# openmm/NNPOps

Hardware: AMD Instinct MI355X
Metric: AEV+forces evaluations/sec (ANI-2x symmetry functions, energy+gradient), 10k-atom periodic box (higher is better)
Workload: dtype f32

## Files before the change

### include/nnpops_hip.h

```cpp
#ifndef NNPOPS_HIP_H
#define NNPOPS_HIP_H

#include <stdint.h>

#ifdef __cplusplus
extern "C" {
#endif

typedef enum {
    NNPOPS_OK = 0,
    NNPOPS_ERR_INVALID_ARGUMENT = -1,
    NNPOPS_ERR_HIP = -2,
    NNPOPS_ERR_UNSUPPORTED = -3,
    NNPOPS_ERR_CAPACITY = -4,
    NNPOPS_ERR_NO_DEVICE = -5
} nnpops_status;

const char* nnpops_last_error(void);
const char* nnpops_version(void);
int nnpops_device_count(void);

typedef struct nnpops_ani* nnpops_ani_t;

int nnpops_ani_create(nnpops_ani_t* out, int num_atoms, int num_species, float radial_cutoff, float angular_cutoff,
// ... 1 lines not shown
                      int num_angular, const float* angular_eta_rs_zeta_ths, int torchani, int device);
int nnpops_ani_destroy(nnpops_ani_t h);
int nnpops_ani_set_stream(nnpops_ani_t h, void* stream);

int nnpops_ani_compute(nnpops_ani_t h, const float* positions, const float* box, float* radial, float* angular);
int nnpops_ani_backprop(nnpops_ani_t h, const float* radial_deriv, const float* angular_deriv, float* position_deriv);
int nnpops_ani_compute_strided(nnpops_ani_t h, const float* positions, const float* box, float* radial, int radial_ld,
                               float* angular, int angular_ld);
int nnpops_ani_backprop_strided(nnpops_ani_t h, const float* radial_deriv, int radial_ld, const float* angular_deriv,
                                int angular_ld, float* position_deriv);
int nnpops_ani_backprop_box_strided(nnpops_ani_t h, const float* positions, const float* box, const float* radial_deriv, int radial_ld,
                                    const float* angular_deriv, int angular_ld, float* position_deriv, float* box_deriv);
int nnpops_ani_tangent_strided(nnpops_ani_t h, const float* position_tangent, float* radial_tangent, int radial_ld,
                               float* angular_tangent, int angular_ld);
int nnpops_ani_check(nnpops_ani_t h, int* max_radial_neighbors, int* max_angular_neighbors);
int nnpops_ani_overflow_word(nnpops_ani_t h, const int32_t** word);
int nnpops_ani_read_overflow(nnpops_ani_t h, int32_t* value);
int nnpops_ani_read_grid(nnpops_ani_t h, int32_t* out);
int nnpops_ani_describe(nnpops_ani_t h, char* text, int capacity);
int nnpops_ani_check_begin(nnpops_ani_t h);
int nnpops_ani_check_begin_with(nnpops_ani_t h, const int32_t** word, int32_t** publish_to, int32_t* stamp);
int nnpops_ani_check_end(nnpops_ani_t h);
int nnpops_ani_set_neighbor_algorithm(nnpops_ani_t h, int algorithm);

int nnpops_ani_set_molecules(nnpops_ani_t h, int num_molecules, const int32_t* molecule_offsets);

enum {
    NNPOPS_ANI_K_NEIGHBORS = 0,
    NNPOPS_ANI_K_RADIAL_FWD = 1,
    NNPOPS_ANI_K_ANGULAR_FWD = 2,
    NNPOPS_ANI_K_RADIAL_BWD = 3,
    NNPOPS_ANI_K_ANGULAR_BWD = 4,
    NNPOPS_ANI_K_CELL_GRID = 5,
    NNPOPS_ANI_NUM_KERNELS = 6
};
int nnpops_ani_enable_timing(nnpops_ani_t h, int enable);
int nnpops_ani_set_timing_stride(nnpops_ani_t h, int every);
int nnpops_ani_get_timing(nnpops_ani_t h, double* total_ms, int* launches);
int nnpops_ani_timing_overhead(nnpops_ani_t h, double* ms);
int nnpops_ani_set_timing_merge(nnpops_ani_t h, int merge);

typedef struct nnpops_cfconv_neighbors* nnpops_cfconv_neighbors_t;
typedef struct nnpops_cfconv* nnpops_cfconv_t;

int nnpops_cfconv_neighbors_create(nnpops_cfconv_neighbors_t* out, int num_atoms, float cutoff, int periodic, int device);
int nnpops_cfconv_neighbors_destroy(nnpops_cfconv_neighbors_t h);
// ... 202 lines not shown
```

### nnpops_amd/capi.py

```python
import ctypes as C
import os

import numpy as np
import torch

_HERE = os.path.dirname(os.path.abspath(__file__))
LIB_PATH = os.path.join(_HERE, "libnnpops_hip.so")

OK = 0
ERR_CAPACITY = -4

SIGNATURES = {
    "nnpops_last_error": (C.c_char_p, []),
    "nnpops_version": (C.c_char_p, []),
    "nnpops_device_count": (C.c_int, []),
    "nnpops_ani_create": (C.c_int, [C.POINTER(C.c_void_p), C.c_int, C.c_int, C.c_float, C.c_float, C.c_int, C.c_void_p,
                                    C.c_int, C.c_void_p, C.c_int, C.c_void_p, C.c_int, C.c_int]),
    "nnpops_ani_destroy": (C.c_int, [C.c_void_p]),
    "nnpops_ani_set_stream": (C.c_int, [C.c_void_p, C.c_void_p]),
    "nnpops_ani_compute": (C.c_int, [C.c_void_p, C.c_void_p, C.c_void_p, C.c_void_p, C.c_void_p]),
    "nnpops_ani_backprop": (C.c_int, [C.c_void_p, C.c_void_p, C.c_void_p, C.c_void_p]),
    "nnpops_ani_compute_strided": (C.c_int, [C.c_void_p, C.c_void_p, C.c_void_p, C.c_void_p, C.c_int, C.c_void_p, C.c_int]),
    "nnpops_ani_backprop_strided": (C.c_int, [C.c_void_p, C.c_void_p, C.c_int, C.c_void_p, C.c_int, C.c_void_p]),
    "nnpops_ani_backprop_box_strided": (C.c_int, [C.c_void_p, C.c_void_p, C.c_void_p, C.c_void_p, C.c_int, C.c_void_p, C.c_int, C.c_void_p,
                                                  C.c_void_p]),
    "nnpops_ani_tangent_strided": (C.c_int, [C.c_void_p, C.c_void_p, C.c_void_p, C.c_int, C.c_void_p, C.c_int]),
    "nnpops_ani_check": (C.c_int, [C.c_void_p, C.POINTER(C.c_int), C.POINTER(C.c_int)]),
    "nnpops_ani_check_begin": (C.c_int, [C.c_void_p]),
    "nnpops_ani_check_end": (C.c_int, [C.c_void_p]),
    "nnpops_ani_set_neighbor_algorithm": (C.c_int, [C.c_void_p, C.c_int]),
    "nnpops_ani_set_molecules": (C.c_int, [C.c_void_p, C.c_int, C.c_void_p]),
    "nnpops_ani_enable_timing": (C.c_int, [C.c_void_p, C.c_int]),
    "nnpops_ani_set_timing_stride": (C.c_int, [C.c_void_p, C.c_int]),
    "nnpops_ani_get_timing": (C.c_int, [C.c_void_p, C.POINTER(C.c_double), C.POINTER(C.c_int)]),
    "nnpops_ani_timing_overhead": (C.c_int, [C.c_void_p, C.POINTER(C.c_double)]),
    "nnpops_ani_overflow_word": (C.c_int, [C.c_void_p, C.POINTER(C.c_void_p)]),
    "nnpops_ani_read_overflow": (C.c_int, [C.c_void_p, C.POINTER(C.c_int32)]),
    "nnpops_ani_read_grid": (C.c_int, [C.c_void_p, C.POINTER(C.c_int32)]),
    "nnpops_ani_describe": (C.c_int, [C.c_void_p, C.c_char_p, C.c_int]),
    "nnpops_ani_check_begin_with": (C.c_int, [C.c_void_p, C.POINTER(C.c_void_p), C.POINTER(C.c_void_p), C.POINTER(C.c_int32)]),
    "nnpops_ani_set_timing_merge": (C.c_int, [C.c_void_p, C.c_int]),
    "nnpops_cfconv_neighbors_create": (C.c_int, [C.POINTER(C.c_void_p), C.c_int, C.c_float, C.c_int, C.c_int]),
    "nnpops_cfconv_neighbors_destroy": (C.c_int, [C.c_void_p]),
    "nnpops_cfconv_neighbors_set_stream": (C.c_int, [C.c_void_p, C.c_void_p]),
    "nnpops_cfconv_neighbors_build": (C.c_int, [C.c_void_p, C.c_void_p, C.c_void_p]),
    "nnpops_cfconv_neighbors_check": (C.c_int, [C.c_void_p, C.POINTER(C.c_int)]),
    "nnpops_cfconv_neighbors_export": (C.c_int, [C.c_void_p, C.c_int, C.c_void_p, C.c_void_p]),
    "nnpops_cfconv_neighbors_read_grid": (C.c_int, [C.c_void_p, C.POINTER(C.c_int32)]),
    "nnpops_cfconv_create": (C.c_int, [C.POINTER(C.c_void_p), C.c_int, C.c_int, C.c_int, C.c_float, C.c_int, C.c_float,
                                       C.c_int, C.c_void_p, C.c_void_p, C.c_void_p, C.c_void_p, C.c_int]),
    "nnpops_cfconv_destroy": (C.c_int, [C.c_void_p]),
    "nnpops_cfconv_set_stream": (C.c_int, [C.c_void_p, C.c_void_p]),
    "nnpops_cfconv_compute": (C.c_int, [C.c_void_p, C.c_void_p, C.c_void_p, C.c_void_p, C.c_void_p, C.c_void_p]),
# ... 183 lines not shown
        self.angular_width = self.num_species * (self.num_species + 1) // 2 * self.num_angular

    def __del__(self):
        h = getattr(self, "_h", None)
        if h:
            self._lib.nnpops_ani_destroy(h)
            self._h = None

    def set_molecules(self, molecule_offsets):
        if molecule_offsets is None:
            _check(self._lib.nnpops_ani_set_molecules(self._h, 0, None))
            self.num_molecules = 0
            return
        off = np.ascontiguousarray(molecule_offsets, dtype=np.int32)
        _check(self._lib.nnpops_ani_set_molecules(self._h, int(off.shape[0]) - 1, off.ctypes.data_as(C.c_void_p)))
        self.num_molecules = int(off.shape[0]) - 1

    def _box_shape(self):
        return (self.num_molecules, 3, 3) if self.num_molecules > 0 else (3, 3)

    def set_neighbor_algorithm(self, algorithm):
        _check(self._lib.nnpops_ani_set_neighbor_algorithm(self._h, int(algorithm)))

    def compute(self, positions, box=None, radial=None, angular=None, check=True):
        _dev_f32(positions, "positions", (self.num_atoms, 3))
        if self.periodic:
            if box is None:
                raise ValueError("periodic evaluator needs box vectors")
            _dev_f32(box, "box", self._box_shape())
        if radial is None:
            radial = torch.empty((self.num_atoms, self.radial_width), dtype=torch.float32, device=positions.device)
        if angular is None:
            angular = torch.empty((self.num_atoms, self.angular_width), dtype=torch.float32, device=positions.device)
        _check(self._lib.nnpops_ani_set_stream(self._h, _stream_ptr(positions.device)))
        for _ in range(8):
            _check(self._lib.nnpops_ani_compute(self._h, _ptr(positions), _ptr(box if self.periodic else None),
                                                _ptr(radial), _ptr(angular)))
            if not check:
                break
            code = self._lib.nnpops_ani_check(self._h, None, None)
            if code == OK:
                break
            if code != ERR_CAPACITY:
                _check(code)
        else:
            raise NNPOpsHipError(ERR_CAPACITY, "neighbour buffers kept overflowing")
# ... 1028 lines not shown
```

### nnpops_amd/csrc/ani.hip

```cpp
#include <algorithm>
#include <cmath>
#include <cstdlib>
#include <cstring>
#include <vector>

#include "ani_kernels.h"
#include "ani_fallback_kernels.h"
#include "ani_angular_mfma.h"
#include "ani_angular_bwd.h"
#include "ani_angular_generic.h"
#include "ani_radial_bwd.h"
#include "ani_build_forward.h"
#include "ani_box_grad.h"
#include "ani_tangent.h"
#include "celllist_host.h"

using namespace nnpops;

constexpr int kRbwdLatencyAtoms = 8192;
constexpr int kFuseAtoms = 4096;
struct nnpops_ani {
    AniParams hp{};
    AngularConsts ac{};
    AniParams* d_params = nullptr;
// ... 43 lines not shown
    int last_compact = -1;
    bool fwd_row_via_lds = true;
    int fwd_occ = 7;
    bool fwd_dynamic = false;
    int nstreams = 1;
    hipStream_t side[3] = {nullptr, nullptr, nullptr};
    hipEvent_t ev_fork = nullptr, ev_join[3] = {nullptr, nullptr, nullptr};
    bool can_split = false;
    int bwd_atoms_per_group = 1;
    int store_mode = 3;
    bool occ6 = false;
    int backward_kernel = 1;
    int fwd_atoms_per_group = 1;
    int* d_cnt_a = nullptr;
    int* d_cnt_ro = nullptr;
    double* d_box_partials = nullptr;
    int* d_status = nullptr;
    int* h_status = nullptr;
    int* h_status_dev = nullptr;
    int check_stamp = 0;
    bool check_pending = false;
    CellList cells;
    bool cells_disabled = false;
    int cap = 0;
    bool cap_fitted = false;
    int cap_angular = 0;
    int tile = 32;
    bool compact_bwd = false;
    bool computed = false;
    int ld_radial = 0, ld_angular = 0;
    bool last_used_cells = false;
    int* d_work_order = nullptr;
    bool work_order_valid = false;
    unsigned char* d_class_tile = nullptr;
    struct BwdClass { int tile, w0, nw; bool two_waves; };
    std::vector<BwdClass> bwd_classes;
    bool bwd_by_class = true;
    bool bwd_two_waves = false;
    double mean_triples = 0;
    int bwd_class_min = 512;
    int bwd_class_atoms = 16384;
    int cell_atoms = 1800;
    int lpt = 2;
    int backprop_stamp = 0;
    unsigned timing_mask = 0;
    int timing_every = 1;
// ... 474 lines not shown
        if (h->mfma_ok) {
            while (hp.fwd_split < 8 && (int)live.size() * hp.fwd_split * 2 <= kFwdSlots) hp.fwd_split *= 2;
            for (size_t b = 0; b < live.size(); b++)
                for (int p = 0; p < hp.fwd_split; p++) hp.fwd_slot_bucket[b * hp.fwd_split + p] = live[b];
        }
        for (int c = 0; c < kMaxAngularFns; c++) hp.m_of_c[c] = -1;
        h->fwd_identity = num_angular == h->nfrp * h->nfzp;
        for (int m = 0; m < num_angular; m++) {
            hp.m_of_c[hp.c_of_m[m]] = m;
            if (hp.c_of_m[m] != m) h->fwd_identity = false;
        }
        hp.fwd_zero_shift = 0;
        while ((4 << hp.fwd_zero_shift) < num_angular && hp.fwd_zero_shift < 6) hp.fwd_zero_shift++;
        h->fwd_identity = h->fwd_identity && num_angular <= 256;
        h->forward_kernel = h->mfma_ok ? 2 : -1;
        if (const char* e = std::getenv("NNPOPS_ANI_FWD_CHUNK")) { h->fwd_chunk = std::min(512, std::max(64, (std::atoi(e) + 15) / 16 * 16)); h->fwd_chunk_forced = true; }
        if (const char* e = std::getenv("NNPOPS_ANI_FUSE")) h->fuse_forward = std::atoi(e) != 0 ? 1 : 0;
        if (const char* e = std::getenv("NNPOPS_ANI_LPT")) h->lpt = std::atoi(e);
        if (const char* e = std::getenv("NNPOPS_ANI_CELL_ATOMS")) h->cell_atoms = std::max(1, std::atoi(e));
        if (const char* e = std::getenv("NNPOPS_ANI_RBWD")) h->rbwd_lanes = std::atoi(e) != 0;
        if (const char* e = std::getenv("NNPOPS_ANI_SCATTER")) h->scatter_mode = std::atoi(e) != 0 ? 1 : 0;
        h->cells.fine = 1;
        if (const char* e = std::getenv("NNPOPS_ANI_FINE_GRID")) h->cells.fine = std::atoi(e) != 0;
        if (const char* e = std::getenv("NNPOPS_ANI_FWD_ROWLDS")) h->fwd_row_via_lds = std::atoi(e) != 0;
        if (const char* e = std::getenv("NNPOPS_ANI_FWD_OCC")) h->fwd_occ = std::atoi(e);
        {
            std::vector<double> frac(num_species, 0.0);
            for (int i = 0; i < num_atoms; i++) frac[atom_species[i]] += 1.0 / num_atoms;
            double fmax = 0;
            for (int a = 0; a < num_species; a++)
                for (int b = a; b < num_species; b++) fmax = std::max(fmax, frac[a] * frac[b] * (a == b ? 1.0 : 2.0));
            h->fwd_dynamic = h->mfma_ok && 32.0 * fmax / hp.fwd_split > 3.0;
        }
        if (const char* e = std::getenv("NNPOPS_ANI_FWD_DYN")) h->fwd_dynamic = std::atoi(e) != 0;
        if (const char* e = std::getenv("NNPOPS_ANI_STREAMS")) h->nstreams = std::max(1, std::min(4, std::atoi(e)));
        if (const char* e = std::getenv("NNPOPS_ANI_BWD_APG")) h->bwd_atoms_per_group = std::atoi(e);
        if (const char* e = std::getenv("NNPOPS_ANI_STORE")) h->store_mode = std::atoi(e) & 3;
        if (const char* e = std::getenv("NNPOPS_ANI_OCC")) h->occ6 = std::atoi(e) >= 6;
        if (const char* e = std::getenv("NNPOPS_ANI_BACKWARD")) { h->backward_kernel = std::min(4, std::max(0, std::atoi(e))); h->backward_forced = true; }
        if (const char* e = std::getenv("NNPOPS_ANI_FWD_WPA")) h->fwd_waves_per_atom = std::atoi(e) == 1 ? 1 : 2;
        if (const char* e = std::getenv("NNPOPS_ANI_FWD_APG")) h->fwd_atoms_per_group = std::max(1, std::atoi(e));
    }
    h->device = device;
    h->cap = 128;
    h->cap_angular = 32;
    if (const char* e = std::getenv("NNPOPS_ANI_CAP")) h->cap = std::max(16, std::atoi(e) & ~15);
// ... 130 lines not shown
            first[m + 1] = (int)blocks.size();
        }
        dev_free(h->d_mol_blocks); dev_free(h->d_mol_first_block); dev_free(h->d_mol_partials);
        h->num_mol_blocks = 0;
        if ((rc = dev_alloc(&h->d_mol_blocks, blocks.size()))) return rc;
        if ((rc = dev_alloc(&h->d_mol_first_block, first.size()))) return rc;
        if ((rc = dev_alloc(&h->d_mol_partials, 9 * blocks.size()))) return rc;
        NNPOPS_HIP_TRY(hipMemcpy(h->d_mol_blocks, blocks.data(), sizeof(int2) * blocks.size(), hipMemcpyHostToDevice));
        NNPOPS_HIP_TRY(hipMemcpy(h->d_mol_first_block, first.data(), sizeof(int) * first.size(), hipMemcpyHostToDevice));
        h->num_mol_blocks = (int)blocks.size();
    }
    h->num_molecules = num_molecules;
    h->computed = false;
    return NNPOPS_OK;
}

int nnpops_ani_set_neighbor_algorithm(nnpops_ani_t h, int algorithm) {
    NNPOPS_REQUIRE(h != nullptr, "NULL handle");
    NNPOPS_REQUIRE(algorithm >= 0 && algorithm <= 2, "algorithm must be 0 (auto), 1 (all pairs) or 2 (cell list)");
    h->algorithm = algorithm;
    return NNPOPS_OK;
}

int nnpops_ani_compute(nnpops_ani_t h, const float* positions, const float* box, float* radial, float* angular) {
    return nnpops_ani_compute_strided(h, positions, box, radial, 0, angular, 0);
}

int nnpops_ani_compute_strided(nnpops_ani_t h, const float* positions, const float* box, float* radial, int radial_ld,
                               float* angular, int angular_ld) {
    NNPOPS_REQUIRE(h != nullptr, "NULL handle");
    {
        const int wr = h->hp.S * h->hp.nR, wa = h->hp.NB * h->hp.nA;
        NNPOPS_REQUIRE((radial_ld == 0 || radial_ld >= wr) && (angular_ld == 0 || angular_ld >= wa),
                       "row strides must be 0 (dense) or at least the row widths (%d, %d)", wr, wa);
        h->ld_radial = radial_ld ? radial_ld : wr;
        h->ld_angular = angular_ld ? angular_ld : wa;
    }
    NNPOPS_REQUIRE(positions && radial && angular, "NULL device pointer");
    NNPOPS_REQUIRE(!h->hp.periodic || box, "periodic handle needs box vectors");
    DeviceGuard guard(h->device);
    if (!guard.ok) return fail(NNPOPS_ERR_HIP, "cannot select device %d", h->device);
    const int N = h->hp.N;
    const bool per = h->hp.periodic;

    const int lds_bw = (int)((builder_lds_bytes(h->cap, h->hp.S, h->hp.NB) + 15) & ~(size_t)15);
    const int wpg_b = waves_per_group(lds_bw);
    const size_t lds_b = (size_t)lds_bw * wpg_b;
    const dim3 ablock(64 * wpg_b);
    const bool use_cells = !h->d_segment && (h->algorithm == 2 || (h->algorithm == 0 && N >= h->cell_atoms && !h->cells_disabled));
    h->last_used_cells = use_cells;
    if (use_cells) {
        KernelTimer timer(h, NNPOPS_ANI_K_CELL_GRID);
        launch_cell_build(h->stream, N, positions, box, per, h->hp.rcr, h->d_species, h->cells);
    }
    h->can_split = !h->generic && h->forward_kernel == 2 && h->backward_kernel >= 1 &&
                   pair_backward_fits(h);
    Span spans[4];
    const int nspans = make_spans(h, spans);
    int rc = fork_streams(h, spans, nspans);
    if (rc != NNPOPS_OK) return rc;
    for (int q = 0; q < nspans; q++) {
        const Span& sp = spans[q];
        const dim3 sgrid(div_up(sp.nw, wpg_b));
        h->last_fused_build = build_forward_fused(h, angular);
        if (h->last_fused_build) {
            KernelTimer timer(h, NNPOPS_ANI_K_NEIGHBORS, sp.stream);
            KernelTimer merged_timer(h, NNPOPS_ANI_K_NEIGHBORS, sp.stream, true);
            const BuildInputs in{box, h->cells.grid, h->cells.cell_start, h->cells.sorted_cell, h->cells.sorted_pos, h->cells.hist, positions, h->d_species,
                                 h->d_segment, use_cells ? 1 : 0, per ? 1 : 0};
            const BuildOutputs out{h->d_nbr, h->d_recA, h->d_recB, h->d_ids, h->d_tri, h->d_cnt_a, h->d_cnt_ro, h->d_cnt_pos, h->d_status, radial, h->ld_radial};
            rc = h->hp.torchani ? launch_build_forward<true>(h, in, out, angular, sp) : launch_build_forward<false>(h, in, out, angular, sp);
            if (rc != NNPOPS_OK) return rc;
            continue;
        }
        KernelTimer merged_timer(h, NNPOPS_ANI_K_NEIGHBORS, sp.stream, true);
// ... 290 lines not shown
                const int tile = tiles[pending];
                h->bwd_classes.push_back({tile, start, end - start, end > start && triples / (end - start) >= 200.0});
                for (int q = start; q < end; q++) tile_of[perm[q]] = (unsigned char)std::min(255, tile);
                start = end;
                pending = c + 1;
            }
        }
        NNPOPS_HIP_TRY(hipMemcpyAsync(h->d_class_tile, tile_of.data(), tile_of.size(), hipMemcpyHostToDevice, h->stream));
        NNPOPS_HIP_TRY(hipStreamSynchronize(h->stream));
        h->work_order_valid = true;
    }
    h->tile = std::min(32, std::max(8, st[kStatMaxAngular]));
    h->compact_bwd = st[kStatMaxAngular] <= h->tile && h->tile >= 16 &&
                     h->tile * (h->tile + 1) + h->tile * (h->tile - 1) / 2 >= h->cap_angular * 4 + 12;
    if (max_radial_neighbors) *max_radial_neighbors = st[kStatMaxRow];
    if (max_angular_neighbors) *max_angular_neighbors = st[kStatMaxAngular];
    if (st[kStatOverflow] == 8) {
        if (!want_order) {
            NNPOPS_HIP_TRY(hipMemset(h->d_class_tile, 255, (size_t)h->hp.N));
            h->bwd_classes.clear();
        }
        return NNPOPS_OK;
    }
    if (st[kStatOverflow] & kGridBinOverflow) {
        int old_bin;
        int rc = h->cells.grow_bins(&old_bin);
        if (rc != NNPOPS_OK) return rc;
        h->computed = false;
        return fail(NNPOPS_ERR_CAPACITY, "cell bins overflowed (%d ids per cell); grown to %d, call compute() again", old_bin, h->cells.bin_cap);
    }
    if (st[kStatOverflow] & kGridBoxTooSmall) {
        if (h->algorithm == 2)
            return fail(NNPOPS_ERR_UNSUPPORTED, "cell list forced but the periodic box is fewer than 3 cells wide on some axis");
        h->cells_disabled = true;
        h->computed = false;
        return fail(NNPOPS_ERR_CAPACITY, "periodic box is fewer than 3 cells wide on some axis: switched to the all-pairs "
                                         "neighbour search, call compute() again");
    }
    if (st[kStatOverflow]) {
        const int old_cap = h->cap, old_ca = h->cap_angular;
        while (h->cap < st[kStatMaxRow]) h->cap *= 2;
        while (h->cap_angular < st[kStatMaxAngular]) h->cap_angular *= 2;
        if (h->cap_angular != old_ca) {
            h->bwd_classes.clear();
            NNPOPS_HIP_TRY(hipMemset(h->d_class_tile, 255, (size_t)h->hp.N));
        }
// ... 29 lines not shown
    return NNPOPS_OK;
}

int nnpops_ani_read_overflow(nnpops_ani_t h, int32_t* value) {
    NNPOPS_REQUIRE(h != nullptr && value != nullptr, "NULL argument");
    DeviceGuard guard(h->device);
    if (!guard.ok) return fail(NNPOPS_ERR_HIP, "cannot select device %d", h->device);
    NNPOPS_HIP_TRY(hipMemcpyAsync(value, h->d_status + kStatOverflow, sizeof(int32_t), hipMemcpyDeviceToHost, h->stream));
    NNPOPS_HIP_TRY(hipStreamSynchronize(h->stream));
    return NNPOPS_OK;
}

int nnpops_ani_read_grid(nnpops_ani_t h, int32_t* out) {
    NNPOPS_REQUIRE(h != nullptr && out != nullptr, "NULL argument");
    DeviceGuard guard(h->device);
    if (!guard.ok) return fail(NNPOPS_ERR_HIP, "cannot select device %d", h->device);
    return h->cells.read_words(h->stream, out);
}

int nnpops_ani_describe(nnpops_ani_t h, char* text, int capacity) {
    NNPOPS_REQUIRE(h != nullptr && text != nullptr && capacity > 0, "NULL argument");
    const bool uni = h->fwd_uniform && h->hp.nFR == h->nfrp && h->hp.nFZ == h->nfzp;
    const bool shape2x = h->nfrp == 8 && h->nfzp == 4;
    std::snprintf(text, (size_t)capacity,
                  "forward=%s backward=%d generic=%d uniform=%d grid=%d literal=%d dynamic_quads=%d fused_build=%d cap=%d cap_angular=%d "
                  "chunk=%d classes=%d cells=%d scatter=%d row_major_walk=%d bwd_mode=%d radial_bwd=%s tile=%d compact=%d%s",
                  h->forward_kernel == 2 ? "mfma" : h->forward_kernel == 1 ? "chunked" : "merge", h->backward_kernel, (int)h->generic,
                  (int)uni, (int)(uni && h->fwd_grid), (int)(uni && h->fwd_grid && shape2x && h->fwd_literal), (int)h->fwd_dynamic,
                  (int)(h->computed ? h->last_fused_build : (h->fuse_forward < 0 ? h->hp.N <= kFuseAtoms : h->fuse_forward != 0)), h->cap, h->cap_angular,
                  h->generic ? h->fwd_chunk : forward_chunk(h, (size_t)h->cap_angular * 2 * sizeof(float4), (size_t)(h->nfrp + h->nfzp) * sizeof(float)),
                  (int)h->bwd_classes.size(), (int)h->last_used_cells,
                  (int)h->scatter_now, h->hp.tri_row_major,
                  h->last_bwd_mode, h->last_radial_lanes < 0 ? "none" : h->last_radial_lanes ? "lanes" : "rows", h->last_tile, h->last_compact,
                  h->hp.periodic && h->d_segment ? " batch_boxes=1" : "");
    return NNPOPS_OK;
}

int nnpops_ani_enable_timing(nnpops_ani_t h, int enable) {
    NNPOPS_REQUIRE(h != nullptr, "NULL handle");
    h->timing_mask = enable == 1 ? ~0u : (unsigned)enable >> 1;
    for (int k = 0; k < NNPOPS_ANI_NUM_KERNELS; k++) { h->ev_used[k] = 0; h->timing_seen[k] = 0; }
    return NNPOPS_OK;
}

int nnpops_ani_set_timing_stride(nnpops_ani_t h, int every) {
    NNPOPS_REQUIRE(h != nullptr, "NULL handle");
    NNPOPS_REQUIRE(every >= 1, "timing stride must be at least 1 (got %d)", every);
    h->timing_every = every;
    return NNPOPS_OK;
}

int nnpops_ani_set_timing_merge(nnpops_ani_t h, int merge) {
    NNPOPS_REQUIRE(h != nullptr, "NULL handle");
    h->timing_merge = merge != 0;
    return NNPOPS_OK;
}
// ... 43 lines not shown
```

### nnpops_amd/csrc/ani_build_forward.h

```cpp
#pragma once

#include "ani_angular_mfma.h"

namespace nnpops {

template <int NFRP, int NFZP>
__host__ __device__ inline size_t build_forward_lds_bytes(int cap, int capA, int S, int NB, int CH, int* tri_offset = nullptr) {
    const size_t recs = (size_t)capA * 2 * sizeof(float4);
    const size_t staging = (size_t)(CH + 1) * (NFRP + NFZP) * sizeof(float) + 64 * sizeof(int);
    const size_t builder = ((builder_lds_bytes(cap, S, NB) + 15) & ~(size_t)15) + 32;
    const size_t mid = ((staging > builder ? staging : builder) + 15) & ~(size_t)15;
    if (tri_offset) *tri_offset = (int)(recs + mid);
    return recs + mid + (size_t)triples_capacity(capA) * sizeof(int);
}

struct BuildInputs {
    const float* box;
    const CellGrid* grid;
    const int* cell_start;
    const int* sorted_cell;
    const float4* sorted_pos;
    int* cell_hist;
    const float* pos;
    const int* species;
// ... 10 lines not shown
};

template <bool TORCHANI, int NFRP, int NFZP, int OCC, int UNI = 0, bool DYN = false>
__global__ __launch_bounds__(128, OCC) void ani_build_forward(const AniParams* __restrict__ P, BuildInputs in, BuildOutputs out, int cap,
                                                              int capA, int CH, float* __restrict__ angular, int ld_angular,
                                                              int vec_ok, int tri_offset, int w0, int nw) {
    extern __shared__ __attribute__((aligned(16))) char lds_raw[];
    const int role = __builtin_amdgcn_readfirstlane(wave_in_group());
    const int lane = lane_id();
    float4* recA_l = (float4*)lds_raw;
    float4* recB_l = recA_l + capA;
    float4* stage = recB_l + capA;
    float* rscratch = (float*)(stage + cap);
    int* groups = (int*)(rscratch + 3 * cap + 64 * P->S);
    const AtomGroups G = carve_groups(groups, P->S, P->NB);
    int* shared = groups + ((group_ints(P->S, P->NB, cap) + 3) & ~(size_t)3);
    int* tri_l = (int*)(lds_raw + tri_offset);
    clear_cell_histogram(in.use_cells ? in.cell_hist : nullptr);

    const float rcr2 = P->rcr2, rca2 = P->rca2;
    Box b{};
    if (in.periodic) b = load_box(in.box);
    CellGrid g{};
    if (in.use_cells) g = *in.grid;

    {
        const int w = blockIdx.x;
        const int slot_id = w0 + w;
        int i = slot_id;
        float4 me = make_float4(0.f, 0.f, 0.f, 0.f);
        const bool void_grid = in.use_cells && !g.ok;
        if (in.use_cells && !void_grid) {
            me = in.sorted_pos[slot_id];
            i = __float_as_int(me.w) & kIdMask;
        } else if (!in.use_cells) {
            me = make_float4(in.pos[3 * i], in.pos[3 * i + 1], in.pos[3 * i + 2], 0.f);
        }
        if (role == 0) {
            int na = 0, nro = 0;
            if (void_grid) {
                if (lane == 0 && slot_id == 0) atomicOr(&out.status[kStatOverflow], refused_grid_bits(g));
            } else if (in.use_cells) {
                const int c = in.sorted_cell[slot_id];
                int cx, cy, cz;
                split_cell(g, c, cx, cy, cz);
                const WideStencil st = gather_wide_stencil(g, in.cell_start, cx, cy, cz);
                int* strip = (int*)rscratch;
// ... 69 lines not shown
```

### nnpops_amd/csrc/ani_kernels.h

```cpp
#pragma once

#include "celllist.h"
#include "device_common.h"

namespace nnpops {

constexpr int kMaxRadialFns = 64;
constexpr int kMaxFactor = 16;
constexpr int kMaxAngularFns = 256;
constexpr int kMaxSpecies = 16;
constexpr int kMaxBuckets = kMaxSpecies * (kMaxSpecies + 1) / 2;
constexpr int kMaxAngularCap = 256;

struct GeoRadial {
    float rs1, c, k1, k0;
    float q, q4, qi4, d4;
};
struct Ani2xAngular {
    static constexpr float zeta = 0x1.c333340000000p+3f, zbias = -0x1.a333340000000p+3f;
    static constexpr float zc0 = 0x1.d906bc0000000p-1f, zc1 = 0x1.87de2a0000000p-2f, zc2 = -0x1.87de280000000p-2f, zc3 = -0x1.d906bc0000000p-1f;
    static constexpr float zs0 = 0x1.87de2c0000000p-2f, zs1 = 0x1.d906bc0000000p-1f, zs2 = 0x1.d906be0000000p-1f, zs3 = 0x1.87de2e0000000p-2f;
    static constexpr float rs_0 = 0x1.99999a0000000p-1f, rs_1 = 0x1.2333340000000p+0f, rs_2 = 0x1.79999a0000000p+0f, rs_3 = 0x1.d000000000000p+0f, rs_4 = 0x1.1333340000000p+1f, rs_5 = 0x1.3e66660000000p+1f, rs_6 = 0x1.69999a0000000p+1f, rs_7 = 0x1.94cccc0000000p+1f;
    static constexpr float negeta = -0x1.9000000000000p+3f;
    static constexpr float rs1 = 0x1.2333340000000p+0f, c = -0x1.2089fc0000000p+4f, k1 = 0x1.8587140000000p+3f, k0 = -0x1.06ee600000000p+1f, q = 0x1.daf9060000000p-5f, q4 = 0x1.7b326e0000000p-17f, qi4 = 0x1.59a8220000000p+16f, d4 = 0x1.5999980000000p+0f;
// ... 375 lines not shown
}

template <bool PERIODIC>
__global__ __launch_bounds__(64 * kWavesPerGroup) void ani_neighbors_cells(const AniParams* __restrict__ P,
                                                          const float* __restrict__ box,
                                                          const CellGrid* __restrict__ grid,
                                                          const int* __restrict__ cell_start,
                                                          const int* __restrict__ sorted_cell,
                                                          const float4* __restrict__ sorted_pos, float4* __restrict__ nbr,
                                                          int cap, int capA, float4* __restrict__ recA,
                                                          float4* __restrict__ recB, int* __restrict__ ids,
                                                          int* __restrict__ tri,
                                                          int* __restrict__ cnt_a, int* __restrict__ cnt_ro, int* __restrict__ cnt_pos,
                                                          int* __restrict__ status, float* __restrict__ radial,
                                                          int ld_radial, int lds_per_wave, int* __restrict__ cell_hist, int slot0, int nslots) {
    extern __shared__ __attribute__((aligned(16))) char lds_raw[];
    float4* stage = (float4*)(lds_raw + (size_t)wave_in_group() * lds_per_wave);
    float* rscratch = (float*)(stage + cap);
    const AtomGroups G = carve_groups((int*)(rscratch + 3 * cap + 64 * P->S), P->S, P->NB);
    const int lane = lane_id();
    const int slot_id = slot0 + wave_global_id();
    clear_cell_histogram(cell_hist);
    if (wave_global_id() >= nslots) return;
    const CellGrid g = *grid;
    if (!g.ok) {
        if (lane == 0) {
            if (slot_id == 0) atomicOr(&status[kStatOverflow], refused_grid_bits(g));
            cnt_a[slot_id] = 0;
            cnt_ro[slot_id] = 0;
            cnt_pos[slot_id] = 0;
        }
        return;
    }
    const float rcr2 = P->rcr2, rca2 = P->rca2;
    Box b{};
    if (PERIODIC) b = load_box(box);
    const float4 me = sorted_pos[slot_id];
    const int c = sorted_cell[slot_id];
    const int i = __float_as_int(me.w) & kIdMask;
    int cx, cy, cz;
    split_cell(g, c, cx, cy, cz);
    float4* row = nbr + (size_t)slot_id * cap;
    int na = 0, nro = 0;
    const WideStencil st = gather_wide_stencil(g, cell_start, cx, cy, cz);
    int* strip = (int*)rscratch;
    int carry = 0;
    constexpr int GROUP = 4;
// ... 68 lines not shown
```

### nnpops_amd/csrc/celllist.h

```cpp
#pragma once

#include "device_common.h"

namespace nnpops {

constexpr int kTagShift = 24;
constexpr int kIdMask = (1 << kTagShift) - 1;

struct CellGrid {
    int nx, ny, nz, ncells;
    int periodic;
    int m;
    int ok;
    int bin_overflow;
    float ox, oy, oz;
    float ixx, iyy, izz;
    float bx, cx, cy;
};

constexpr int kGridBoxTooSmall = 2;
constexpr int kGridBinOverflow = 4;
__device__ __forceinline__ int refused_grid_bits(const CellGrid& g) {
    return g.bin_overflow ? (kGridBoxTooSmall | kGridBinOverflow) : kGridBoxTooSmall;
}
// ... 277 lines not shown
    const int i = blockIdx.x * kBinnedThreads + threadIdx.x;
    const int ic = min(i, N - 1);
    const float x = pos[3 * ic], y = pos[3 * ic + 1], z = pos[3 * ic + 2];
    if (threadIdx.x == 0) {
        g = decide_grid(1, box, nullptr, nullptr, cutoff, min(max_cells, kBinnedCells), fine);
        if (blockIdx.x == 0) *grid = g;
    }
    __syncthreads();
    const int c = bin_one_atom(i, N, g, x, y, z, hist, bins, bin_cap);
    if (c >= 0) atom_cell[i] = c;
}

template <int T>
static __global__ __launch_bounds__(T) void order_binned(int N, const float* __restrict__ pos,
                                                                      const int* __restrict__ tag, CellGrid* __restrict__ grid,
                                                                      const int* __restrict__ hist,
                                                                      const int* __restrict__ bins, int bin_cap,
                                                                      const int* __restrict__ atom_cell, int* __restrict__ cell_start,
                                                                      int* __restrict__ sorted_atom, float4* __restrict__ sorted_pos,
                                                                      int* __restrict__ sorted_cell) {
    __shared__ int s_start[kBinnedCells + 1];
    __shared__ int wave_tot[T / 64];
    order_block<T>(N, grid, pos, tag, hist, bins, bin_cap, atom_cell, cell_start, sorted_atom, sorted_pos, sorted_cell, s_start, wave_tot);
}

constexpr int kStencilRanges = 18;
struct Stencil {
    int pre[kStencilRanges];
    int delta;
    int total;
};

__device__ __forceinline__ Stencil gather_stencil(const CellGrid& g, const int* __restrict__ cell_start, int cx, int cy, int cz) {
    const int lane = lane_id();
    int begin = 0, end = 0;
    if (lane < kStencilRanges) {
        const int pair = lane >> 1, sub = lane & 1;
        int z = cz + pair / 3 - 1, y = cy + pair % 3 - 1;
        bool live = true;
        if (g.periodic) { z = (z + g.nz) % g.nz; y = (y + g.ny) % g.ny; }
        else live = z >= 0 && z < g.nz && y >= 0 && y < g.ny;
        if (live) {
            const int rowbase = (z * g.ny + y) * g.nx;
            int x0 = cx - 1, x1 = cx + 1, a = 0, b = -1;
            if (!g.periodic) { if (sub == 0) { a = max(x0, 0); b = min(x1, g.nx - 1); } }
            else if (x0 < 0) { if (sub == 0) { a = b = g.nx - 1; } else { a = 0; b = x1; } }
// ... 171 lines not shown
    for (int q = 1; q < kStencilCells; q++) r += k >= S.pre[q] ? 1 : 0;
    return k + __builtin_amdgcn_ds_bpermute(r << 2, S.delta);
}

__device__ __forceinline__ void clear_cell_histogram(int* __restrict__ hist) {
    if (hist == nullptr) return;
    const int stride = gridDim.x * blockDim.x;
    for (int c = blockIdx.x * blockDim.x + threadIdx.x; c < kHistWords; c += stride) hist[c] = 0;
}

struct CellBuffers {
    CellGrid* grid = nullptr;
    int *cell_count = nullptr, *cell_start = nullptr;
    int *atom_cell = nullptr, *atom_rank = nullptr;
    int *unsorted_atom = nullptr, *sorted_atom = nullptr;
    float4* sorted_pos = nullptr;
    int max_cells = 0;
    int* hist = nullptr;
    int* bins = nullptr;
    int bin_cap = 0;
    int fine = 0;
    int* sorted_cell = nullptr;
    int* tile_total = nullptr;
};

static inline void grid_words(const CellGrid& g, int32_t* out) {
    out[0] = g.nx; out[1] = g.ny; out[2] = g.nz; out[3] = g.ncells;
    out[4] = g.m; out[5] = g.ok; out[6] = g.bin_overflow; out[7] = g.periodic;
}

static inline bool cell_build_is_binned(int N, bool periodic, const CellBuffers& b) {
    return periodic && b.hist != nullptr && b.bins != nullptr;
}

static inline void launch_cell_build(hipStream_t stream, int N, const float* pos, const float* box, bool periodic, float cutoff,
                                     const int* tag, const CellBuffers& b) {
    const int tb = 256, nb = (N + tb - 1) / tb;
    if (cell_build_is_binned(N, periodic, b)) {
        hipLaunchKernelGGL(bin_atoms, dim3(nb), dim3(kBinnedThreads), 0, stream, N, pos, box, cutoff, b.max_cells, b.grid, b.hist, b.bins,
                           b.bin_cap, b.atom_cell, b.fine);
        hipLaunchKernelGGL(order_binned<kBinnedThreads>, dim3(nb), dim3(kBinnedThreads), 0, stream, N, pos, tag, b.grid, b.hist, b.bins, b.bin_cap,
                           b.atom_cell, b.cell_start, b.sorted_atom, b.sorted_pos, b.sorted_cell);
        return;
    }
    hipLaunchKernelGGL(grid_setup, dim3(periodic ? 32 : 1), dim3(256), 0, stream, N, pos, box, (int)periodic, cutoff, b.max_cells, b.grid, b.cell_count, b.fine);
    hipLaunchKernelGGL(assign_cells, dim3(nb), dim3(tb), 0, stream, N, pos, b.grid, b.cell_count, b.atom_cell, b.atom_rank);
    if (b.max_cells <= kScanTile || b.tile_total == nullptr) {
        hipLaunchKernelGGL(scan_cells, dim3(1), dim3(1024), 0, stream, b.grid, b.cell_count, b.cell_start, (int*)nullptr);
    } else {
        const int ntiles = (b.max_cells + kScanTile - 1) / kScanTile;
        hipLaunchKernelGGL(scan_cells, dim3(ntiles), dim3(1024), 0, stream, b.grid, b.cell_count, b.cell_start, b.tile_total);
        hipLaunchKernelGGL(add_tile_offsets, dim3(ntiles), dim3(1024), 0, stream, b.grid, b.tile_total, b.cell_start);
    }
    hipLaunchKernelGGL(fill_cells, dim3(nb), dim3(tb), 0, stream, N, b.grid, b.cell_start, b.atom_cell, b.atom_rank, b.unsorted_atom);
    hipLaunchKernelGGL(order_cells, dim3(nb), dim3(tb), 0, stream, N, pos, b.grid, b.cell_start, b.atom_cell, b.unsorted_atom, tag,
                       b.sorted_atom, b.sorted_pos, b.sorted_cell);
}

template <typename F>
__device__ __forceinline__ void for_each_stencil_range(const CellGrid& g, const int* __restrict__ cell_start, int cx,
// ... 29 lines not shown
```

### nnpops_amd/csrc/celllist_host.h

```cpp
#pragma once

#include <algorithm>
#include <cstdlib>

#include "celllist.h"
#include "host_common.h"

namespace nnpops {

inline int read_grid_words(const CellGrid* d_grid, hipStream_t stream, int32_t* out) {
    CellGrid g;
    NNPOPS_HIP_TRY(hipMemcpyAsync(&g, d_grid, sizeof(CellGrid), hipMemcpyDeviceToHost, stream));
    NNPOPS_HIP_TRY(hipStreamSynchronize(stream));
    grid_words(g, out);
    return NNPOPS_OK;
}

struct CellList : CellBuffers {
    static int cells_for(int N) { return N + 4096; }
    static size_t tile_total_len(int max_cells) { return (size_t)max_cells / kScanTile + 2; }

    template <typename F>
    int each_array(size_t n, bool binned, bool tiled_scan, F&& f) {
        int rc = NNPOPS_OK;
        auto visit = [&](auto*& p, size_t len) { if (rc == NNPOPS_OK) rc = f(p, len); };
        visit(grid, 1);
        visit(cell_count, (size_t)max_cells);
        visit(cell_start, (size_t)max_cells + 1);
        visit(atom_cell, n);
        visit(atom_rank, n);
        visit(unsorted_atom, n);
        visit(sorted_atom, n);
        visit(sorted_pos, n);
        visit(sorted_cell, n);
        if (binned) { visit(hist, (size_t)kHistWords); visit(bins, (size_t)kBinnedCells * bin_cap); }
        if (tiled_scan) visit(tile_total, tile_total_len(max_cells));
        return rc;
    }

    int allocate(int N, bool periodic, bool tiled_scan) {
        max_cells = cells_for(N);
        bin_cap = 64;
        if (const char* e = std::getenv("NNPOPS_CELL_BIN_CAP")) bin_cap = std::max(4, std::atoi(e) & ~3);
        const bool binned = periodic && N <= kBinnedAtoms;
        int rc = each_array((size_t)N, binned, tiled_scan, [](auto*& p, size_t len) { return dev_alloc(&p, len); });
        if (rc != NNPOPS_OK) return rc;
        if (binned && hipMemset(hist, 0, sizeof(int) * kHistWords) != hipSuccess) return fail(NNPOPS_ERR_HIP, "memset failed");
        return NNPOPS_OK;
    }

    void release() {
        each_array(0, true, true, [](auto*& p, size_t) { dev_free(p); return (int)NNPOPS_OK; });
    }

    int grow_bins(int* old_cap) {
        *old_cap = bin_cap;
        bin_cap *= 2;
        dev_free(bins);
        return dev_alloc(&bins, (size_t)kBinnedCells * bin_cap);
    }

    int read_words(hipStream_t stream, int32_t* out) const { return read_grid_words(grid, stream, out); }
};

}
```

Baseline: 12260.

## Build periodic cell grid in one kernel launch with per-block owned cell ranges

Adds a single-launch cell-list build for periodic systems of up to 20k atoms. Each block recomputes the grid, scans all positions to count atoms before its z-slab range, stages candidates in LDS, then computes cell starts and the sorted order for the cells it owns. This replaces the two-launch binned build and cuts launch count and inter-kernel gaps. In exchange every block rereads all positions, and a capacity overflow now forces a fallback and a retry of compute(). It is enabled by default.

```diff
diff --git a/include/nnpops_hip.h b/include/nnpops_hip.h
--- a/include/nnpops_hip.h
+++ b/include/nnpops_hip.h
@@ -47,6 +47,7 @@
 int nnpops_ani_check_begin_with(nnpops_ani_t h, const int32_t** word, int32_t** publish_to, int32_t* stamp);
 int nnpops_ani_check_end(nnpops_ani_t h);
 int nnpops_ani_set_neighbor_algorithm(nnpops_ani_t h, int algorithm);
+int nnpops_ani_set_grid_build(nnpops_ani_t h, int one_launch);
 
 int nnpops_ani_set_molecules(nnpops_ani_t h, int num_molecules, const int32_t* molecule_offsets);
 
diff --git a/nnpops_amd/capi.py b/nnpops_amd/capi.py
--- a/nnpops_amd/capi.py
+++ b/nnpops_amd/capi.py
@@ -29,6 +29,7 @@
     "nnpops_ani_check_begin": (C.c_int, [C.c_void_p]),
     "nnpops_ani_check_end": (C.c_int, [C.c_void_p]),
     "nnpops_ani_set_neighbor_algorithm": (C.c_int, [C.c_void_p, C.c_int]),
+    "nnpops_ani_set_grid_build": (C.c_int, [C.c_void_p, C.c_int]),
     "nnpops_ani_set_molecules": (C.c_int, [C.c_void_p, C.c_int, C.c_void_p]),
     "nnpops_ani_enable_timing": (C.c_int, [C.c_void_p, C.c_int]),
     "nnpops_ani_set_timing_stride": (C.c_int, [C.c_void_p, C.c_int]),
@@ -258,6 +259,9 @@
     def set_neighbor_algorithm(self, algorithm):
         _check(self._lib.nnpops_ani_set_neighbor_algorithm(self._h, int(algorithm)))
 
+    def set_grid_build(self, one_launch):
+        _check(self._lib.nnpops_ani_set_grid_build(self._h, int(bool(one_launch))))
+
     def compute(self, positions, box=None, radial=None, angular=None, check=True):
         _dev_f32(positions, "positions", (self.num_atoms, 3))
         if self.periodic:
diff --git a/nnpops_amd/csrc/ani.hip b/nnpops_amd/csrc/ani.hip
--- a/nnpops_amd/csrc/ani.hip
+++ b/nnpops_amd/csrc/ani.hip
@@ -89,6 +89,7 @@
     bool check_pending = false;
     CellList cells;
     bool cells_disabled = false;
+    int last_grid_build = -1;
     int cap = 0;
     bool cap_fitted = false;
     int cap_angular = 0;
@@ -609,6 +610,9 @@
         if (const char* e = std::getenv("NNPOPS_ANI_SCATTER")) h->scatter_mode = std::atoi(e) != 0 ? 1 : 0;
         h->cells.fine = 1;
         if (const char* e = std::getenv("NNPOPS_ANI_FINE_GRID")) h->cells.fine = std::atoi(e) != 0;
+        h->cells.owned = 1;
+        if (const char* e = std::getenv("NNPOPS_ANI_GRID_OWNED")) h->cells.owned = std::atoi(e) != 0;
+        if (const char* e = std::getenv("NNPOPS_ANI_GRID_BLOCKS")) h->cells.owned_launch = std::max(kOwnedMinBlocks, std::min(256, std::atoi(e)));
         if (const char* e = std::getenv("NNPOPS_ANI_FWD_ROWLDS")) h->fwd_row_via_lds = std::atoi(e) != 0;
         if (const char* e = std::getenv("NNPOPS_ANI_FWD_OCC")) h->fwd_occ = std::atoi(e);
         {
@@ -785,6 +789,15 @@
     return NNPOPS_OK;
 }
 
+int nnpops_ani_set_grid_build(nnpops_ani_t h, int one_launch) {
+    NNPOPS_REQUIRE(h != nullptr, "NULL handle");
+    DeviceGuard guard(h->device);
+    if (!guard.ok) return fail(NNPOPS_ERR_HIP, "cannot select device %d", h->device);
+    h->cells.owned = one_launch != 0;
+    if (h->cells.owned) NNPOPS_HIP_TRY(hipMemsetAsync(&h->cells.grid->bin_overflow, 0, sizeof(int), h->stream));
+    return NNPOPS_OK;
+}
+
 int nnpops_ani_compute(nnpops_ani_t h, const float* positions, const float* box, float* radial, float* angular) {
     return nnpops_ani_compute_strided(h, positions, box, radial, 0, angular, 0);
 }
@@ -814,6 +827,7 @@
     h->last_used_cells = use_cells;
     if (use_cells) {
         KernelTimer timer(h, NNPOPS_ANI_K_CELL_GRID);
+        h->last_grid_build = cell_build_is_owned(N, per, h->cells) ? 2 : cell_build_is_binned(N, per, h->cells) ? 1 : 0;
         launch_cell_build(h->stream, N, positions, box, per, h->hp.rcr, h->d_species, h->cells);
     }
     h->can_split = !h->generic && h->forward_kernel == 2 && h->backward_kernel >= 1 &&
@@ -1150,6 +1164,12 @@
         }
         return NNPOPS_OK;
     }
+    if ((st[kStatOverflow] & kGridBinOverflow) && h->last_grid_build == 2) {
+        h->cells.owned = 0;
+        h->computed = false;
+        return fail(NNPOPS_ERR_CAPACITY, "a cell range of the one-launch grid build holds more than %d atoms: switched to the two-launch build, "
+                                         "call compute() again", kOwnedCap);
+    }
     if (st[kStatOverflow] & kGridBinOverflow) {
         int old_bin;
         int rc = h->cells.grow_bins(&old_bin);
@@ -1225,9 +1245,10 @@
     NNPOPS_REQUIRE(h != nullptr && text != nullptr && capacity > 0, "NULL argument");
     const bool uni = h->fwd_uniform && h->hp.nFR == h->nfrp && h->hp.nFZ == h->nfzp;
     const bool shape2x = h->nfrp == 8 && h->nfzp == 4;
+    const bool grid_next = !h->d_segment && (h->algorithm == 2 || (h->algorithm == 0 && h->hp.N >= h->cell_atoms && !h->cells_disabled));
     std::snprintf(text, (size_t)capacity,
                   "forward=%s backward=%d generic=%d uniform=%d grid=%d literal=%d dynamic_quads=%d fused_build=%d cap=%d cap_angular=%d "
-                  "chunk=%d classes=%d cells=%d scatter=%d row_major_walk=%d bwd_mode=%d radial_bwd=%s tile=%d compact=%d%s",
+                  "chunk=%d classes=%d cells=%d scatter=%d row_major_walk=%d bwd_mode=%d radial_bwd=%s tile=%d compact=%d%s%s%s",
                   h->forward_kernel == 2 ? "mfma" : h->forward_kernel == 1 ? "chunked" : "merge", h->backward_kernel, (int)h->generic,
                   (int)uni, (int)(uni && h->fwd_grid), (int)(uni && h->fwd_grid && shape2x && h->fwd_literal), (int)h->fwd_dynamic,
                   (int)(h->computed ? h->last_fused_build : (h->fuse_forward < 0 ? h->hp.N <= kFuseAtoms : h->fuse_forward != 0)), h->cap, h->cap_angular,
@@ -1235,6 +1256,8 @@
                   (int)h->bwd_classes.size(), (int)h->last_used_cells,
                   (int)h->scatter_now, h->hp.tri_row_major,
                   h->last_bwd_mode, h->last_radial_lanes < 0 ? "none" : h->last_radial_lanes ? "lanes" : "rows", h->last_tile, h->last_compact,
+                  grid_next ? " grid_build=" : "",
+                  !grid_next ? "" : !h->hp.periodic || !h->cells.hist ? "scan" : cell_build_is_owned(h->hp.N, true, h->cells) ? "owned" : "binned",
                   h->hp.periodic && h->d_segment ? " batch_boxes=1" : "");
     return NNPOPS_OK;
 }
diff --git a/nnpops_amd/csrc/ani_build_forward.h b/nnpops_amd/csrc/ani_build_forward.h
--- a/nnpops_amd/csrc/ani_build_forward.h
+++ b/nnpops_amd/csrc/ani_build_forward.h
@@ -56,7 +56,7 @@
     Box b{};
     if (in.periodic) b = load_box(in.box);
     CellGrid g{};
-    if (in.use_cells) g = *in.grid;
+    if (in.use_cells) g = load_built_grid(in.grid);
 
     {
         const int w = blockIdx.x;
diff --git a/nnpops_amd/csrc/ani_kernels.h b/nnpops_amd/csrc/ani_kernels.h
--- a/nnpops_amd/csrc/ani_kernels.h
+++ b/nnpops_amd/csrc/ani_kernels.h
@@ -421,7 +421,7 @@
     const int slot_id = slot0 + wave_global_id();
     clear_cell_histogram(cell_hist);
     if (wave_global_id() >= nslots) return;
-    const CellGrid g = *grid;
+    const CellGrid g = load_built_grid(grid);
     if (!g.ok) {
         if (lane == 0) {
             if (slot_id == 0) atomicOr(&status[kStatOverflow], refused_grid_bits(g));
diff --git a/nnpops_amd/csrc/celllist.h b/nnpops_amd/csrc/celllist.h
--- a/nnpops_amd/csrc/celllist.h
+++ b/nnpops_amd/csrc/celllist.h
@@ -323,6 +323,190 @@
     __shared__ int s_start[kBinnedCells + 1];
     __shared__ int wave_tot[T / 64];
     order_block<T>(N, grid, pos, tag, hist, bins, bin_cap, atom_cell, cell_start, sorted_atom, sorted_pos, sorted_cell, s_start, wave_tot);
+}
+
+constexpr int kOwnedThreads = 1024;
+constexpr int kOwnedMinBlocks = 32, kOwnedMaxBlocks = 128;
+constexpr int kOwnedMaxPer = kBinnedCells / kOwnedMinBlocks;
+constexpr int kOwnedCap = 2 * kOwnedThreads;
+constexpr int kOwnedMaybe = 2304;
+constexpr int kOwnedUnroll = 10;
+constexpr int kOwnedAtoms = 20000;
+
+static inline int owned_blocks(int N) {
+    const int b = (N + 127) / 128;
+    return b < kOwnedMinBlocks ? kOwnedMinBlocks : b > kOwnedMaxBlocks ? kOwnedMaxBlocks : b;
+}
+
+__device__ __forceinline__ CellGrid load_built_grid(const CellGrid* __restrict__ grid) {
+    CellGrid g = *grid;
+    if (g.bin_overflow) g.ok = 0;
+    return g;
+}
+
+__device__ __forceinline__ int cell_slab(const CellGrid& g, float z) {
+    float sz = (z - g.oz) * g.izz;
+    if (g.periodic) sz -= floorf(sz);
+    return min(max((int)(sz * g.nz), 0), g.nz - 1);
+}
+
+struct PackedPos { float x, y, z; };
+
+static __global__ __launch_bounds__(kOwnedThreads) void bin_atoms_owned(int N, const float* __restrict__ pos,
+                                                                         const int* __restrict__ tag,
+                                                                         const float* __restrict__ box, float cutoff, int max_cells,
+                                                                         CellGrid* __restrict__ grid, int* __restrict__ atom_cell,
+                                                                         int* __restrict__ cell_start, int* __restrict__ sorted_atom,
+                                                                         float4* __restrict__ sorted_pos, int* __restrict__ sorted_cell,
+                                                                         int fine) {
+    constexpr int T = kOwnedThreads, U = kOwnedUnroll, WAVES = T / 64;
+    __shared__ CellGrid g;
+    __shared__ float4 s_maybe[kOwnedMaybe];
+    __shared__ int s_own[kOwnedCap];
+    __shared__ int s_key[kOwnedCap];
+    __shared__ int s_bucket[kOwnedCap];
+    __shared__ int s_cnt[kOwnedMaxPer];
+    __shared__ int s_start[kOwnedMaxPer];
+    __shared__ int s_n, s_nm, s_zlo, s_zhi;
+    __shared__ int wave_tot[WAVES], wave_before[WAVES];
+    const int tid = threadIdx.x, lane = tid & 63, wave = tid >> 6;
+    const PackedPos* __restrict__ p3 = reinterpret_cast<const PackedPos*>(pos);
+    PackedPos p[U];
+#pragma unroll
+    for (int u = 0; u < U; u++) p[u] = p3[min(tid + u * T, N - 1)];
+    if (tid < kOwnedMaxPer) s_cnt[tid] = 0;
+    if (tid == 0) {
+        s_n = 0;
+        s_nm = 0;
+        g = decide_grid(1, box, nullptr, nullptr, cutoff, min(max_cells, kBinnedCells), fine);
+        if (blockIdx.x == 0) {
+            grid->nx = g.nx; grid->ny = g.ny; grid->nz = g.nz; grid->ncells = g.ncells;
+            grid->periodic = g.periodic; grid->m = g.m; grid->ok = g.ok;
+            grid->ox = g.ox; grid->oy = g.oy; grid->oz = g.oz;
+            grid->ixx = g.ixx; grid->iyy = g.iyy; grid->izz = g.izz;
+            grid->bx = g.bx; grid->cx = g.cx; grid->cy = g.cy;
+        }
+        const int nxy = g.nx * g.ny, per0 = (g.ncells + (int)gridDim.x - 1) / (int)gridDim.x;
+        const int lo = min((int)blockIdx.x * per0, g.ncells), hi = min(lo + per0, g.ncells);
+        s_zlo = lo / nxy;
+        s_zhi = (max(hi, 1) - 1) / nxy;
+    }
+    __syncthreads();
+    if (!g.ok) return;
+    const int ncells = g.ncells;
+    const int per = (ncells + (int)gridDim.x - 1) / (int)gridDim.x;
+    const int c0 = min((int)blockIdx.x * per, ncells), c1 = min(c0 + per, ncells);
+    if (c0 >= c1) return;
+    const int zlo = s_zlo, zhi = s_zhi;
+
+    int before = 0;
+    for (int base = tid;;) {
+        unsigned mask = 0;
+#pragma unroll
+        for (int u = 0; u < U; u++) {
+            const int z = (base + u * T < N) ? cell_slab(g, p[u].z) : g.nz;
+            before += z < zlo ? 1 : 0;
+            mask |= (z >= zlo && z <= zhi) ? 1u << u : 0u;
+        }
+        {
+            const int cnt = __popc(mask), incl = wave_prefix_sum(cnt);
+            int room = 0;
+            if (lane == 63 && incl > 0) room = atomicAdd(&s_nm, incl);
+            int at = __builtin_amdgcn_readlane(room, 63) + incl - cnt;
+#pragma unroll
+            for (int u = 0; u < U; u++)
+                if (mask >> u & 1) {
+                    if (at < kOwnedMaybe) s_maybe[at] = make_float4(p[u].x, p[u].y, p[u].z, __int_as_float(base + u * T));
+                    at++;
+                }
+        }
+        base += U * T;
+        if (base - tid >= N) break;
+#pragma unroll
+        for (int u = 0; u < U; u++) p[u] = p3[min(base + u * T, N - 1)];
+    }
+    __syncthreads();
+    const int nm = s_nm;
+    if (nm > kOwnedMaybe) {
+        if (tid == 0) grid->bin_overflow = 1;
+        return;
+    }
+    {
+        constexpr int R = (kOwnedMaybe + T - 1) / T;
+#pragma unroll
+        for (int r = 0; r < R; r++)
+            if (tid + r * T < nm) {
+                const float4 m = s_maybe[tid + r * T];
+                int cx, cy, cz;
+                cell_of(g, m.x, m.y, m.z, cx, cy, cz);
+                const int c = (cz * g.ny + cy) * g.nx + cx;
+                before += c < c0 ? 1 : 0;
+                if (c >= c0 && c < c1) {
+                    const int k = atomicAdd(&s_cnt[c - c0], 1);
+                    const int e = atomicAdd(&s_n, 1);
+                    if (e < kOwnedCap) {
+                        s_own[e] = tid + r * T;
+                        s_key[e] = ((c - c0) << 16) | k;
+                    }
+                }
+            }
+    }
+    {
+        const int incl = wave_prefix_sum(before);
+        if (lane == 63) wave_before[wave] = incl;
+    }
+    __syncthreads();
+    const int n = s_n;
+    if (n > kOwnedCap) {
+        if (tid == 0) grid->bin_overflow = 1;
+        return;
+    }
+    float mx[2], my[2], mz[2];
+    int id[2], key[2], tg[2];
+#pragma unroll
+    for (int q = 0; q < 2; q++) {
+        const int e = min(tid + q * T, max(n - 1, 0));
+        const float4 m = s_maybe[n > 0 ? s_own[e] : 0];
+        mx[q] = m.x; my[q] = m.y; mz[q] = m.z;
+        id[q] = __float_as_int(m.w);
+        key[q] = s_key[e];
+        tg[q] = (tag && tid + q * T < n) ? tag[id[q]] : 0;
+    }
+    int count = 0, incl = 0;
+    if (tid < kOwnedMaxPer) {
+        count = s_cnt[tid];
+        incl = wave_prefix_sum(count);
+        if (lane == 63) wave_tot[wave] = incl;
+    }
+    int first = 0;
+#pragma unroll
+    for (int w = 0; w < WAVES; w++) first += wave_before[w];
+    __syncthreads();
+    if (tid < kOwnedMaxPer) {
+        int start = incl - count;
+        for (int w = 0; w < wave; w++) start += wave_tot[w];
+        s_start[tid] = start;
+        if (c0 + tid < c1) cell_start[c0 + tid] = first + start;
+    }
+    if (tid == 0 && c1 == ncells && c0 < c1) cell_start[ncells] = N;
+    __syncthreads();
+#pragma unroll
+    for (int q = 0; q < 2; q++)
+        if (tid + q * T < n) s_bucket[s_start[key[q] >> 16] + (key[q] & 0xffff)] = id[q];
+    __syncthreads();
+#pragma unroll
+    for (int q = 0; q < 2; q++) {
+        if (tid + q * T >= n) continue;
+        const int lc = key[q] >> 16, i = id[q];
+        const int lo = s_start[lc], cnt = s_cnt[lc];
+        int rank = 0;
+        for (int a = 0; a < cnt; a++) rank += s_bucket[lo + a] < i ? 1 : 0;
+        const int slot = first + lo + rank;
+        sorted_atom[slot] = i;
+        if (sorted_cell) sorted_cell[slot] = c0 + lc;
+        sorted_pos[slot] = make_float4(mx[q], my[q], mz[q], __int_as_float(i | (tg[q] << kTagShift)));
+        atom_cell[i] = c0 + lc;
+    }
 }
 
 constexpr int kStencilRanges = 18;
@@ -540,20 +724,31 @@
     int fine = 0;
     int* sorted_cell = nullptr;
     int* tile_total = nullptr;
+    int owned = 0;
+    int owned_launch = 0;
 };
 
 static inline void grid_words(const CellGrid& g, int32_t* out) {
     out[0] = g.nx; out[1] = g.ny; out[2] = g.nz; out[3] = g.ncells;
-    out[4] = g.m; out[5] = g.ok; out[6] = g.bin_overflow; out[7] = g.periodic;
+    out[4] = g.m; out[5] = g.bin_overflow ? 0 : g.ok; out[6] = g.bin_overflow; out[7] = g.periodic;
 }
 
 static inline bool cell_build_is_binned(int N, bool periodic, const CellBuffers& b) {
     return periodic && b.hist != nullptr && b.bins != nullptr;
+}
+
+static inline bool cell_build_is_owned(int N, bool periodic, const CellBuffers& b) {
+    return b.owned != 0 && N <= kOwnedAtoms && cell_build_is_binned(N, periodic, b);
 }
 
 static inline void launch_cell_build(hipStream_t stream, int N, const float* pos, const float* box, bool periodic, float cutoff,
                                      const int* tag, const CellBuffers& b) {
     const int tb = 256, nb = (N + tb - 1) / tb;
+    if (cell_build_is_owned(N, periodic, b)) {
+        hipLaunchKernelGGL(bin_atoms_owned, dim3(b.owned_launch > 0 ? b.owned_launch : owned_blocks(N)), dim3(kOwnedThreads), 0, stream, N, pos, tag, box,
+                           cutoff, b.max_cells, b.grid, b.atom_cell, b.cell_start, b.sorted_atom, b.sorted_pos, b.sorted_cell, b.fine);
+        return;
+    }
     if (cell_build_is_binned(N, periodic, b)) {
         hipLaunchKernelGGL(bin_atoms, dim3(nb), dim3(kBinnedThreads), 0, stream, N, pos, box, cutoff, b.max_cells, b.grid, b.hist, b.bins,
                            b.bin_cap, b.atom_cell, b.fine);
diff --git a/nnpops_amd/csrc/celllist_host.h b/nnpops_amd/csrc/celllist_host.h
--- a/nnpops_amd/csrc/celllist_host.h
+++ b/nnpops_amd/csrc/celllist_host.h
@@ -45,6 +45,7 @@
         const bool binned = periodic && N <= kBinnedAtoms;
         int rc = each_array((size_t)N, binned, tiled_scan, [](auto*& p, size_t len) { return dev_alloc(&p, len); });
         if (rc != NNPOPS_OK) return rc;
+        if (hipMemset(grid, 0, sizeof(CellGrid)) != hipSuccess) return fail(NNPOPS_ERR_HIP, "memset failed");
         if (binned && hipMemset(hist, 0, sizeof(int) * kHistWords) != hipSuccess) return fail(NNPOPS_ERR_HIP, "memset failed");
         return NNPOPS_OK;
     }
```

After: 12540, median of 6. +2.2%, better.
